# SaeedRahmani/AV-Simulation-at-Intersections

Hardware: AMD Instinct MI355X
Metric: MPC steps/sec (batch x horizon) at N=20 nu=2 (higher is better)
Workload: dtype f64

## Files before the change

av-simulation-at-intersections_amd/csrc/jsim_mpc.hip:

```cpp
#include <hip/hip_runtime.h>
#include <dlfcn.h>

#include <algorithm>
#include <cmath>
#include <cstdarg>
#include <cstdint>
#include <cstdio>
#include <cstdlib>
#include <cstring>
#include <new>
#include <type_traits>
#include <vector>

#include "jsim_mpc.h"

#define JSIM_VIOL_TOL 1e-10
#define JSIM_KEY_MASK 0xFFFFF
__device__ __forceinline__ double jsim_key_trunc(double k)
{
    return __hiloint2double(__double2hiint(k), __double2loint(k) & ~JSIM_KEY_MASK);
}
__device__ __forceinline__ double jsim_ratio_trunc(double t)
{
    return __hiloint2double(__double2hiint(t), __double2loint(t) & ~127);
// ... 9 lines not shown
#define JSIM_DEP_TOL 1e-18
#define JSIM_ACT_TOL 1e-9
#define JSIM_FEAS_TOL 1e-8

typedef double v4d __attribute__((ext_vector_type(4)));

struct KP {
    int T, n, ld, B;
    int pass;
    double dt, dl, L, w_perp, w_para;
    double R0, R1, Rd0, Rd1, Qv, Qyaw, Qf0, Qf1, Qf2, Qf3, Re0, Re1;
    double dmax, amax, amin, smax, vmax_plant, vmin, vref_min;
    double jerkw;
    const double2 *pxy;
    const double *pyaw;
    const double *pcv;
    const int *cv_cut;
    const double *pe;
    const long long *poff;
    const double *x0;
    const int *path_id;
    const int *path_len;
    const double *speed;
    long long *target_ind;
    double *oa, *od, *ox, *oy, *ov, *oyaw, *xref;
    unsigned *amask;
    int *status;
    int *n_iter;
    double *dbg_xbar;
    long long *dbg_idx;
// ... 1144 lines not shown
    {
        if (grew) *grew = n > cap;
        if (n <= cap) return hipSuccess;
        release();
        const hipError_t e = hipMalloc(&p, sizeof(T) * n);
        if (e == hipSuccess) cap = n; else p = nullptr;
        return e;
    }
};

struct jsim_ctx {
    jsim_cfg cfg{};
    int device = 0;
    DevArray<double2> d_pxy;
    DevArray<double> d_pyaw;
    DevArray<long long> d_poff;
    int n_paths = 0;
    long long n_points = 0;
    double *h_cx = nullptr, *h_cy = nullptr, *h_cyaw = nullptr;
    int have_geom = 0;
    double cc0 = 0, cc1 = 0, col_radius = 0;
    DevArray<double> d_get_all;
    DevArray<double2> d_pred_all;
    DevArray<double4> d_bc_all;
    DevArray<double4> d_pred_bc;
    double occ0 = 0, occ1 = 0, ocol_radius = 0, oL = 0;
    int have_ogeom = 0;
    DevArray<double4> d_shapes;
    DevArray<double2> d_othr;
    std::vector<double> h_shapes;
// ... 144 lines not shown
    jsim_ctx *c = new (std::nothrow) jsim_ctx();
    if (!c) return fail(nullptr, -12, "jsim_mpc_create: out of memory");
    c->cfg = *cfg;
    c->device = device_id;
    c->lds_bytes = lds_bytes;
    const char *force = getenv("JSIM_FORCE_LDS_KERNEL");
    c->use_reg_kernel = cfg->nx == 4 && has_reg_kernel(cfg->T) && !(force && force[0] == '1');
    const char *mg = getenv("JSIM_DEBUG_MAX_GI");
    c->dbg_max_gi = mg ? atoi(mg) : -1;
    *out = c;
    return 0;
}

static void free_paths(jsim_ctx *c)
{
    c->d_pxy.release(); c->d_pyaw.release(); c->d_poff.release(); c->d_pcc.release(); c->d_pcv.release();
    delete[] c->h_cx; delete[] c->h_cy; delete[] c->h_cyaw;
    c->h_cx = c->h_cy = c->h_cyaw = nullptr;
    c->n_paths = 0; c->n_points = 0;
}

extern "C" void jsim_mpc_destroy(jsim_ctx *ctx)
{
    if (!ctx) return;
    if (ctx->comm) (void)jsim_comm_destroy(ctx);
    DeviceGuard dev_guard(ctx->device);
    free_paths(ctx);
    delete ctx;
}

static int upload_circle_centres(jsim_ctx *ctx)
{
    const long long N = ctx->n_points;
    if (N <= 0 || !ctx->h_cx) return 0;
    std::vector<double2> h((size_t)2 * N);
    for (long long i = 0; i < N; ++i) {
        const double c = std::cos(ctx->h_cyaw[i]), s = std::sin(ctx->h_cyaw[i]);
        h[2 * i].x = c * ctx->cc0 - s * 0.0 + ctx->h_cx[i];     h[2 * i].y = s * ctx->cc0 + c * 0.0 + ctx->h_cy[i];
        h[2 * i + 1].x = c * ctx->cc1 - s * 0.0 + ctx->h_cx[i]; h[2 * i + 1].y = s * ctx->cc1 + c * 0.0 + ctx->h_cy[i];
    }
    ctx->d_pcc.release();
    HIP_TRY(ctx, ctx->d_pcc.reserve(2 * N));
    HIP_TRY(ctx, hipMemcpy(ctx->d_pcc, h.data(), sizeof(double2) * 2 * N, hipMemcpyHostToDevice));
    return 0;
}

extern "C" int jsim_mpc_set_paths(jsim_ctx *ctx, const double *cx, const double *cy, const double *cyaw,
                                  const int64_t *path_off, int32_t n_paths)
{
    if (!ctx) return fail(nullptr, -22, "jsim_mpc_set_paths: null ctx");
    DeviceGuard dev_guard(ctx->device);
    JSIM_GUARD_OK(ctx);
    if (!cx || !cy || !cyaw || !path_off || n_paths < 1) return fail(ctx, -22, "jsim_mpc_set_paths: bad argument");
    if (path_off[0] != 0) return fail(ctx, -22, "jsim_mpc_set_paths: path_off[0] must be 0");
    for (int i = 0; i < n_paths; ++i)
        if (path_off[i + 1] <= path_off[i]) return fail(ctx, -22, "jsim_mpc_set_paths: path %d is empty", i);
    const long long N = path_off[n_paths];
    free_paths(ctx);
    double2 *h = new (std::nothrow) double2[N];
    if (!h) return fail(ctx, -12, "jsim_mpc_set_paths: out of host memory");
    for (long long i = 0; i < N; ++i) { h[i].x = cx[i]; h[i].y = cy[i]; }
    hipError_t e = ctx->d_pxy.reserve(N);
    if (e == hipSuccess) e = ctx->d_pyaw.reserve(N);
    if (e == hipSuccess) e = ctx->d_poff.reserve(n_paths + 1);
    if (e == hipSuccess) e = hipMemcpy(ctx->d_pxy, h, sizeof(double2) * N, hipMemcpyHostToDevice);
    if (e == hipSuccess) e = hipMemcpy(ctx->d_pyaw, cyaw, sizeof(double) * N, hipMemcpyHostToDevice);
    if (e == hipSuccess) e = hipMemcpy(ctx->d_poff, path_off, sizeof(long long) * (n_paths + 1), hipMemcpyHostToDevice);
    delete[] h;
    if (e != hipSuccess) { free_paths(ctx); return fail(ctx, -5, "jsim_mpc_set_paths: %s", hipGetErrorString(e)); }
    ctx->n_paths = n_paths;
    ctx->n_points = N;
    ctx->h_cx = new (std::nothrow) double[N]; ctx->h_cy = new (std::nothrow) double[N]; ctx->h_cyaw = new (std::nothrow) double[N];
    if (!ctx->h_cx || !ctx->h_cy || !ctx->h_cyaw) return fail(ctx, -12, "jsim_mpc_set_paths: out of host memory");
    memcpy(ctx->h_cx, cx, sizeof(double) * N); memcpy(ctx->h_cy, cy, sizeof(double) * N); memcpy(ctx->h_cyaw, cyaw, sizeof(double) * N);
    if (ctx->have_geom) return upload_circle_centres(ctx);
    return 0;
}

struct StepBufs {
    double *x0; const int32_t *path_id, *path_len; const double *speed; int64_t *target_ind;
    double *oa, *od, *ox, *oy, *ov, *oyaw, *xref; uint32_t *active_mask; int32_t *status, *n_iter;
};
struct AdvanceBufs {
// ... 41 lines not shown
}

static KP fill_kp(const jsim_ctx *ctx, int32_t B, const StepBufs &S)
{
    const jsim_cfg &c = ctx->cfg;
    KP P;
    memset(&P, 0, sizeof(P));
    P.T = c.T; P.n = jsim_nvar(c.T, c.nx == 5); P.ld = jsim_ld(P.n); P.B = B;
    P.jerkw = c.jerk_weight;
    P.dt = c.dt; P.dl = c.dl; P.L = c.L; P.w_perp = c.w_perp; P.w_para = c.w_para;
    P.R0 = c.R[0]; P.R1 = c.R[1]; P.Rd0 = c.Rd[0]; P.Rd1 = c.Rd[1]; P.Qv = c.Q_v_yaw[0]; P.Qyaw = c.Q_v_yaw[1];
    P.Qf0 = c.Qf[0] * c.T; P.Qf1 = c.Qf[1] * c.T; P.Qf2 = c.Qf[2] * c.T; P.Qf3 = c.Qf[3] * c.T;
    P.Re0 = c.R_end[0]; P.Re1 = c.R_end[1];
    P.dmax = c.max_dsteer * c.dt; P.amax = c.max_accel; P.amin = c.max_decel; P.smax = c.max_steer;
    P.vmax_plant = c.max_speed; P.vmin = c.min_speed; P.vref_min = c.min_ref_speed;
    P.pxy = ctx->d_pxy; P.pyaw = ctx->d_pyaw; P.poff = ctx->d_poff;
    P.pcv = ctx->d_pcv; P.cv_cut = ctx->cv_cut; P.pe = ctx->d_pe;
    P.x0 = S.x0; P.path_id = S.path_id; P.path_len = S.path_len; P.speed = S.speed;
    P.target_ind = (long long *)S.target_ind; P.oa = S.oa; P.od = S.od; P.ox = S.ox; P.oy = S.oy; P.ov = S.ov; P.oyaw = S.oyaw;
    P.xref = S.xref; P.amask = S.active_mask; P.status = S.status; P.n_iter = S.n_iter;
    P.dbg_clk = ctx->dbg_clk; P.dbg_max_gi = ctx->dbg_max_gi;
    return P;
}

static double jsim_sqrt_threshold(double thr)
{
    double x = thr * thr;
    while (std::sqrt(x) > thr) x = std::nextafter(x, 0.0);
    while (std::sqrt(std::nextafter(x, INFINITY)) <= thr) x = std::nextafter(x, INFINITY);
    return x;
}
// ... 1136 lines not shown
```

av-simulation-at-intersections_amd/csrc/mpc_step_reg.inc:

```

template <int CTRL>
__device__ __forceinline__ double dpp_f64(double v)
{
    int lo = __double2loint(v), hi = __double2hiint(v);
    lo = __builtin_amdgcn_update_dpp(0, lo, CTRL, 0xf, 0xf, true);
    hi = __builtin_amdgcn_update_dpp(0, hi, CTRL, 0xf, 0xf, true);
    return __hiloint2double(hi, lo);
}
template <int CTRL>
__device__ __forceinline__ int dpp_i32(int v) { return __builtin_amdgcn_update_dpp(0, v, CTRL, 0xf, 0xf, true); }

#define DPP_QP_1032 0xB1
#define DPP_QP_2301 0x4E
#define DPP_ROW_HALF_MIRROR 0x141
#define DPP_ROW_MIRROR 0x140
#define DPP_ROW_SHR(n) (0x110 + (n))

__device__ __forceinline__ double wsum_dpp(double v)
{
    v += dpp_f64<DPP_QP_1032>(v);
    v += dpp_f64<DPP_QP_2301>(v);
    v += dpp_f64<DPP_ROW_HALF_MIRROR>(v);
    v += dpp_f64<DPP_ROW_MIRROR>(v);
    return (rdlane(v, 0) + rdlane(v, 16)) + (rdlane(v, 32) + rdlane(v, 48));
// ... 295 lines not shown
    if ((int)blockIdx.x >= Pin.B) return;
    const int ego = K.order ? K.order[blockIdx.x] : (int)blockIdx.x;
    if (Pin.pe) jsim_apply_ego_cfg(P, Pin.pe, ego, Pin.T, Pin.dt);
    constexpr int N = 2 * T, NR = 3 * T + 1, LD = N + 1, TP = T + 2, MW = (8 * T + 31) / 32;
    constexpr int NTILE = (N + 15) / 16;
    constexpr bool VS = NR >= 64;
    constexpr int NW = VS ? N : NR;
    static_assert(NW < 64, "register path needs 2T+1 lanes (3T+2 with resident speed rows)");
    constexpr int NP = N + 2;
    constexpr int LDC = N + 2, CCH = 16;
    constexpr bool LCA = VS || (WPE == 2 && T > 13);
    constexpr int HLN = LCA ? N * LDC : N * LD + N * LDC;
    constexpr int PREN = PRE ? (int)((sizeof(PreScratch) + 7) / 8) : 0;
    __shared__ __attribute__((aligned(16))) double HL[HLN > PREN ? HLN : PREN];
    double *const Hm = HL;
    double *const Lc = HL + (LCA ? 0 : N * LD);
    static_assert((N * LD) % 2 == 0, "Lc stays 16-byte aligned");
    __shared__ __attribute__((aligned(16))) double gsv[2 * N];
    __shared__ __attribute__((aligned(16))) double drow12[2 * NP];
    double *const drow = drow12, *const drow2 = drow12 + NP;
    __shared__ __attribute__((aligned(16))) double dzv[NP];
    __shared__ __attribute__((aligned(16))) double vzv[NP];
    __shared__ __attribute__((aligned(16))) double rdv[NP];
    __shared__ __attribute__((aligned(16))) double UV[VS ? 2 : NR + 5];
    constexpr int TQN = (TQ_COUNT * TP + 1) & ~1 ;
    constexpr int SPH = (T + 1) & ~1, SPN = VS ? T * SPH : 0;
    static_assert(!VS || (SPN >= NR + 5 || TQN + 3 * NP >= NR + 5), "uvec fits the shared area");
    __shared__ __attribute__((aligned(16))) double SCR[(TQN + 3 * NP > SPN) ? TQN + 3 * NP : SPN];
    double *const tq = SCR, *const invc = SCR + TQN, *const gvc = SCR + TQN + NP, *const wvc = SCR + TQN + 2 * NP;
    double *const spdump = SCR;
// ... 78 lines not shown
                    if (lane0 == 0) { hb_rd[(hwave - 1) * 3 + r] = v; hb_ri[(hwave - 1) * 3 + r] = id; }
                    if (i0 == id) { b0 = b1; i0 = i1; b1 = b2; i1 = i2; b2 = INFINITY; i2 = 0x7fffffff; }
                }
            } else if (cmd == HB_HBUILD) {
                if (hwave == 1 && NTILE > 1) jsim_h_tile_row<T, 1>(tq, Hm, lane0, dt);
                else if (hwave == 2 && NTILE > 2) jsim_h_tile_row<T, 2>(tq, Hm, lane0, dt);
                else if (hwave == 3 && NTILE > 3) jsim_h_tile_row<T, 3>(tq, Hm, lane0, dt);
                if (hwave == 3) { const double gi = jsim_g_own<T>(tq, lane0, dt); if (lane0 < N) gvc[lane0] = gi; }
            } else if (cmd == HB_JBUILD && hwave == 1) {
                double Jr[N];
#define JSIM_J_WAIT(n_) jsim_spin_published(&invc[(n_) - 1])
#include "mpc_step_reg_j.inc"
#undef JSIM_J_WAIT
#pragma unroll
                for (int j = 0; j < N; j += 2) *(double2 *)&Jx[lane0 * (N + 2) + j] = double2{Jr[j], Jr[j + 1]};
            }
            __syncthreads();
        }
    }
    for (int tk = 0; tk < K.n_ticks; ++tk) {
    if (WPE == 2) {
        sx = uni(sx); sy = uni(sy); sv = uni(sv); syaw = uni(syaw); di_prev = uni(di_prev); ai_last = uni(ai_last);
        goal_xy.x = uni(goal_xy.x); goal_xy.y = uni(goal_xy.y); s0 = uni64(s0); age = uni(age);
    }
#define LANE_FENCE() do { lane = lane0; asm volatile("" : "+v"(lane)); __builtin_assume(lane >= 0 && lane < 64); } while (0)
    LANE_FENCE();
    if (PRE) {
        PreScratch &W = *reinterpret_cast<PreScratch *>(HL);
        PreP pre = Q.pre;
        pre.n_obs = pre_obs.n;
        const PreOut o = jsim_pre_tick_ego(pre, Q.pred_cc_all + ((size_t)tk * Q.pre.n_obs + pre_obs.first) * Q.pre.n_steps * 2,
                                           Q.pred_bc_all + (size_t)tk * Q.pre.n_obs + pre_obs.first, pre_othr, W, lane, ego,
                                           off, Mfull, sx, sy, sv, pre_idx, pre_prev);
        pre_st = o.status;
        if (o.status == JSIM_OK) {
            pre_idx = o.idx; pre_col = o.col;
            if (Q.speed_cutoff) pre_cut = o.path_len; else M = o.path_len;
        }
        pre_prev = Q.speed_cutoff ? Mfull : (int)M;
        LDS_SYNC();
        LANE_FENCE();
    }
    double a0n = 0.0, d0n = 0.0;
    int status = JSIM_OK;
    int hp = 0;
    bool s2_done = false;
    do {
    STAMP(0);
    double bx = sx, by = sy, bv = sv, bth = syaw, sn, cs;
    long long tind = s0;
    {
        long long len = M - s0;
        if (len < 0) len = 0;
        if (M < 1) {
            status = 3;
        } else if (len >= 3) {
            double b0 = INFINITY, b1 = INFINITY, b2 = INFINITY;
            int i0 = 0x7fffffff, i1 = 0x7fffffff, i2 = 0x7fffffff;
            const double2 *pp = P.pxy + off + s0;
            const int ilen = (int)len;
#define INSERT_PT(p_, k_)                                                                      \
// ... 47 lines not shown
            tind = s0 + 1;
        }
    }
    if (status != JSIM_OK) {
        if (lane == 0) {
            P.status[ego] = status;
            if (P.n_iter) P.n_iter[ego] = it_base;
        }
        break;
    }

    STAMP(1);
    LANE_FENCE();
    const int tl_idx = lane < T ? lane : T;
    double xr, yr, yawr, vr = 0.0;
    bool rend;
    long long ik;
    {
        const double vref = (P.vref_min > sv) ? P.vref_min : sv;
        const double cstep = fabs(vref) * dt;
        double trav = cstep;
        if (P.pass == 0) {
#pragma unroll
            for (int j = 1; j <= T; ++j)
                if (j <= tl_idx) trav = trav + cstep;
        } else {
            const double *ovp = P.ov + (size_t)ego * (T + 1);
            trav = fabs(ovp[0]) * dt;
#pragma unroll
            for (int j = 1; j <= T; ++j)
                if (j <= tl_idx) trav = trav + fabs(ovp[j]) * dt;
        }
        ik = (long long)rint(trav / P.dl) + tind;
        if (ik > M - 1) ik = M - 1;
        const double2 pr = P.pxy[off + ik];
        xr = pr.x; yr = pr.y; yawr = P.pyaw[off + ik];
        rend = (ik == M - 1);
        if (P.pcv) {
            const int cut = (PRE && Q.speed_cutoff) ? pre_cut : (P.cv_cut ? P.cv_cut[ego] : -1);
            vr = (cut < 0 || ik < cut) ? P.pcv[off + ik] : 0.0;
        }
    }
    if (speed - sv < -JSIM_FEAS_TOL || sv - P.vmin < -JSIM_FEAS_TOL) status = JSIM_INFEASIBLE;

    STAMP(2);
    LANE_FENCE();
    if (!(HELP && s2_done)) {
#include "mpc_step_reg_s2.inc"
    }
    if (P.dbg_xbar && lane <= T) {
        double *xb = P.dbg_xbar + (size_t)ego * 4 * (T + 1);
        xb[0 * (T + 1) + lane] = bx; xb[1 * (T + 1) + lane] = by;
        xb[2 * (T + 1) + lane] = bv; xb[3 * (T + 1) + lane] = bth;
    }
    if (P.dbg_idx && lane <= T) P.dbg_idx[(size_t)ego * (T + 1) + lane] = ik;
    if (P.xref && lane <= T) {
        double *xf = P.xref + (size_t)ego * 4 * (T + 1);
        xf[0 * (T + 1) + lane] = xr; xf[1 * (T + 1) + lane] = yr;
        xf[2 * (T + 1) + lane] = vr; xf[3 * (T + 1) + lane] = yawr;
    }
    if (status == JSIM_INFEASIBLE) {
        if (tl) { P.oa[(size_t)ego * T + lane] = 0.0; P.od[(size_t)ego * T + lane] = 0.0; }
        wa_t = 0.0; wd_t = 0.0; s0 = tind;
        if (P.amask && lane < MW) P.amask[(size_t)ego * MW + lane] = 0u;
        if (lane == 0) {
            P.status[ego] = status;
            P.target_ind[ego] = tind;
            if (P.n_iter) P.n_iter[ego] = it_base;
        }
        break;
    }

    STAMP(3);
    LANE_FENCE();
    double al = 0, be = 0, alp = 0, bep = 0, ccx = 0, ccy = 0, kt = 0;
    if (tl) {
        al = dt * cs;
        be = (-dt * bv) * sn;
        alp = dt * sn;
        bep = (dt * bv) * cs;
        ccx = ((dt * bv) * sn) * bth;
        ccy = ((-dt * bv) * cs) * bth;
        kt = (dt * bv) / P.L;
    }
    {
        const double PA = wexscan_dpp(al, lane), PB = wexscan_dpp(be, lane);
        const double PAP = wexscan_dpp(alp, lane), PBP = wexscan_dpp(bep, lane);
        const double FX = sx + wexscan_dpp(fma(al, sv, fma(be, syaw, ccx)), lane);
        const double FY = sy + wexscan_dpp(fma(alp, sv, fma(bep, syaw, ccy)), lane);
        double Qxx = 0, Qxy = 0, Qyy = 0, qv = 0, qyaw = 0;
        if (lane >= 1 && lane <= T) {
            if (!rend) {
                const double a1 = yawr + 0.5 * M_PI;
                double c1, s1, c2, s2;
                sincos(a1, &s1, &c1); sincos(yawr, &s2, &c2);
                Qxx = (c1 * c1) * P.w_perp + (c2 * c2) * P.w_para;
                Qxy = (c1 * s1) * P.w_perp + (c2 * s2) * P.w_para;
                Qyy = (s1 * s1) * P.w_perp + (s2 * s2) * P.w_para;
                qv = P.Qv; qyaw = P.Qyaw;
            } else {
                Qxx = P.Qf0; Qyy = P.Qf1; qv = P.Qf2; qyaw = P.Qf3;
            }
        }
        const double ex = FX - xr, ey = FY - yr, ev = sv - vr, eyaw = syaw - yawr;
        if (lane <= T + 1) {
            const int t = lane;
            const bool in = lane <= T;
            tq[TQ_PA * TP + t] = PA; tq[TQ_PB * TP + t] = PB; tq[TQ_PAP * TP + t] = PAP; tq[TQ_PBP * TP + t] = PBP;
            tq[TQ_KT * TP + t] = kt;
            tq[TQ_QXX * TP + t] = in ? Qxx : 0; tq[TQ_QXY * TP + t] = in ? Qxy : 0; tq[TQ_QYY * TP + t] = in ? Qyy : 0;
// ... 245 lines not shown
        }
        LDS_SYNC();
        {
            const int rb = evl ? (lane >> 1) * NP : 0;
            double n0 = 0.0, n1 = 0.0;
#pragma unroll
            for (int j = 0; j < N; j += 2) {
                const double2 p2 = *(const double2 *)&HL[rb + j];
                n0 = fma(p2.x, p2.x, n0); n1 = fma(p2.y, p2.y, n1);
            }
            spw = (dt * dt) * (n0 + n1);
        }
        LDS_SYNC();
    }
    double *const Rm = Hm;
    for (int e = lane; e < N * LD; e += 64) Rm[e] = 0.0;
    if (lane < N) { gsv[2 * lane] = 1.0; gsv[2 * lane + 1] = 0.0; }
    if (lane < 2) { drow[N + lane] = 0.0; drow2[N + lane] = 0.0; dzv[N + lane] = 0.0; vzv[N + lane] = 0.0; }
    LDS_SYNC();

    STAMP(9);
    LANE_FENCE();
    int cid0 = -1, cid1 = -1, cid2 = -1, cid3 = -1;
    double ub0 = 0.0, lb1 = 0.0;
    const double dmx = P.dmax;
    double thr0 = 0, thr1 = 0, thr23 = 0;
    double ub2 = dmx, lb3 = -dmx, thr3 = 0;
    if (lane < N) {
        const int t = lane >> 1;
        if ((lane & 1) == 0) {
            cid0 = 4 * T + t; cid1 = 5 * T + t;
            ub0 = P.amax; lb1 = P.amin;
            thr0 = JSIM_VIOL_TOL * (1.0 + fabs(P.amax)); thr1 = JSIM_VIOL_TOL * (1.0 + fabs(P.amin));
// ... 6 lines not shown
            cid0 = 6 * T + 2 * t; cid1 = cid0 + 1;
            ub0 = P.smax; lb1 = -P.smax;
            thr0 = thr1 = JSIM_VIOL_TOL * (1.0 + P.smax);
            if (t + 1 < T) { cid2 = 2 * t; cid3 = 2 * t + 1; }
            thr23 = thr3 = JSIM_VIOL_TOL * (1.0 + P.dmax);
        }
    } else if (!VS && lane < NR && lane > N) {
        const int t = lane - N;
        cid0 = 2 * T - 2 + t; cid1 = 3 * T - 1 + t;
        ub0 = speed; lb1 = P.vmin;
        thr0 = JSIM_VIOL_TOL * (1.0 + fabs(speed - sv)); thr1 = JSIM_VIOL_TOL * (1.0 + fabs(sv - P.vmin));
    }
    double iw01, iw23, w01, w23;
    {
        double rn0 = 0.0, rn1 = 0.0, dn0 = 0.0, dn1 = 0.0;
#pragma unroll
        for (int j = 0; j < N; j += 2) {
            rn0 = fma(Jr[j], Jr[j], rn0); rn1 = fma(Jr[j + 1], Jr[j + 1], rn1);
            const double e0 = __shfl_down(Jr[j], 2) - Jr[j], e1 = __shfl_down(Jr[j + 1], 2) - Jr[j + 1];
            dn0 = fma(e0, e0, dn0); dn1 = fma(e1, e1, dn1);
        }
        const double rn = rn0 + rn1;
        const double dn = (VS && lane < N && !(lane & 1)) ? spw : dn0 + dn1;
        w01 = rn > 0.0 ? rn : 1.0;
        w23 = dn > 0.0 ? dn : 1.0;
        iw01 = fast_rcp(w01);
        iw23 = fast_rcp(w23);
    }

    int q = 0, iters = 0;
    constexpr int max_iters = 50 * N + 100;
#ifdef JSIM_STAMPS
    long long gclk[8] = {0, 0, 0, 0, 0, 0, 0, 0}, gt0 = 0, gt1 = 0;
#define GSTAMP0() do { gt0 = (long long)__builtin_readcyclecounter(); } while (0)
#define GSTAMP(i) do { gt1 = (long long)__builtin_readcyclecounter(); gclk[i] += gt1 - gt0; gt0 = gt1; } while (0)
// ... 346 lines not shown
    }
#undef JSIM_SEARCH
#undef JSIM_SEARCH_A
#undef JSIM_SEARCH_B1
#undef JSIM_SEARCH_B2
#undef JSIM_SEARCH_C

    STAMP(10);
#ifdef JSIM_STAMPS
    if (P.dbg_clk && lane == 0)
        for (int i_ = 0; i_ < 8; ++i_) P.dbg_clk[(size_t)P.B * 16 + (size_t)ego * 8 + i_] = gclk[i_];
#endif
    LANE_FENCE();
    if (status != JSIM_OK) {
        if (tl) { P.oa[(size_t)ego * T + lane] = 0.0; P.od[(size_t)ego * T + lane] = 0.0; }
        wa_t = 0.0; wd_t = 0.0; s0 = tind;
        if (P.amask && lane < MW) P.amask[(size_t)ego * MW + lane] = 0u;
        if (lane == 0) {
            P.status[ego] = status;
            P.target_ind[ego] = tind;
            if (P.n_iter) P.n_iter[ego] = it_base + iters;
            if (K.work) K.work[ego] += (unsigned)iters;
            if (K.iters) K.iters[ego] += (unsigned long long)iters;
        }
        break;
    }
    if (lane < MW) maskw[lane] = 0u;
    if (lane < (VS ? N : NR)) uvec[lane] = val;
    if (VS) {
        const bool evl = lane < N && !(lane & 1);
        const double vsp = fma(dt, wincscan_dpp(evl ? val : 0.0, lane), sv);
// ... 13 lines not shown
        if (P.amask && lane < MW) P.amask[(size_t)ego * MW + lane] = maskw[lane];
    }
    {
        double a = 0.0, dl_ = 0.0;
        if (tl) { a = uvec[2 * lane]; dl_ = uvec[2 * lane + 1]; }
        const double vt = lane <= T ? uvec[N + lane] : sv;
        if (PARK && lane <= T) {
            al = tq[TQ_QXX * TP + lane]; be = tq[TQ_QXY * TP + lane]; alp = tq[TQ_QYY * TP + lane];
            bep = tq[TQ_QV * TP + lane]; ccx = tq[TQ_QYAW * TP + lane]; ccy = tq[TQ_QEX * TP + lane]; kt = tq[TQ_KT * TP + lane];
        }
        const double yt = syaw + wexscan_dpp(kt * dl_, lane);
        const double xt = sx + wexscan_dpp(fma(al, vt, fma(be, yt, ccx)), lane);
        const double yy = sy + wexscan_dpp(fma(alp, vt, fma(bep, yt, ccy)), lane);
        if (tl) { P.oa[(size_t)ego * T + lane] = a; P.od[(size_t)ego * T + lane] = dl_; }
        wa_t = a; wd_t = dl_; s0 = tind;
        a0n = uvec[0]; d0n = uvec[1];
        if (lane <= T) {
            const size_t o = (size_t)ego * (T + 1) + lane;
            if (P.ox) P.ox[o] = xt;
            if (P.oy) P.oy[o] = yy;
            if (P.ov) P.ov[o] = vt;
            if (P.oyaw) P.oyaw[o] = yt;
        }
    }
    if (lane == 0) {
        P.status[ego] = JSIM_OK;
        P.target_ind[ego] = tind;
        if (P.n_iter) P.n_iter[ego] = it_base + iters;
        if (K.work) K.work[ego] += (unsigned)iters;
        if (K.iters) K.iters[ego] += (unsigned long long)iters;
// ... 11 lines not shown
        double di = di_prev, ai;
        if (status == JSIM_OK) { di = d0n; ai = a0n; }
        else ai = P.amin;
        di_prev = di;
        ai_last = ai;
        if (K.hist && lane == 0) {
            const int k = hist_base + tk;
            if (k < K.hist_cap) { K.hist[((size_t)k * P.B + ego) * 2] = di; K.hist[((size_t)k * P.B + ego) * 2 + 1] = ai; }
        }
        if (K.rec && lane == 0 && *K.tick + tk < K.rec_cap)
            jsim_rec_store_dev(K.rec, *K.tick + tk, P.B, ego,
                               status == JSIM_OK ? jsim_xref_deviation(P.pxy[off + s0], P.pyaw[off + s0], sx, sy) : __builtin_nan(""));
        double dc = (P.smax < di) ? P.smax : di;
        dc = (-P.smax > dc) ? -P.smax : dc;
        double cy_, sy_;
        sincos(syaw, &sy_, &cy_);
        const double xd = sv * cy_, yd = sv * sy_, thd = (sv / P.L) * tan(dc);
        sx += xd * dt; sy += yd * dt; syaw += thd * dt;
        sv += ai * dt;
        sv = (P.vmax_plant < sv) ? P.vmax_plant : sv;
        sv = (P.vmin > sv) ? P.vmin : sv;
        bool isgoal = hypot(sx - goal_xy.x, sy - goal_xy.y) <= K.goal_dis;
        long long df = s0 - M;
        if ((df < 0 ? -df : df) >= 5) isgoal = false;
        const bool done = (isgoal && fabs(sv) <= K.stop_speed) || (age + 1 >= K.max_age);
        if (K.rec && lane == 0) {
            const int k = *K.tick + tk;
            if (k < K.rec_cap)
                jsim_rec_store(K.rec, K.rec_flags, k, P.B, ego, sx, sy, syaw, sv, di, ai,
                               (status == JSIM_OK ? 0 : JSIM_REC_FAILED) | (isgoal && fabs(sv) <= K.stop_speed ? JSIM_REC_GOAL : 0) |
                                   (age + 1 >= K.max_age ? JSIM_REC_AGE : 0));
        }
        if (done) {
            sx = K.x0_spawn[4 * ego]; sy = K.x0_spawn[4 * ego + 1]; sv = K.x0_spawn[4 * ego + 2]; syaw = K.x0_spawn[4 * ego + 3];
            s0 = K.target_spawn[ego];
            wa_t = 0.0; wd_t = 0.0; di_prev = 0.0; ai_last = 0.0; age = 0;
            if (PRE) { pre_idx = 0; pre_prev = -1; }
            if (tl) { P.oa[(size_t)ego * T + lane] = 0.0; P.od[(size_t)ego * T + lane] = 0.0; }
            if (lane == 0) {
                P.target_ind[ego] = s0;
                if (K.n_respawn) atomicAdd(K.n_respawn, 1ull);
            }
        } else {
            age += 1;
        }
    }
    LDS_SYNC();
    }
    if (HELP) {
        if (lane0 == 0) hb_cmd = HB_EXIT;
        __syncthreads();
// ... 16 lines not shown
```

av-simulation-at-intersections_amd/csrc/mpc_step_reg4.inc:

```

__host__ __device__ constexpr int jsim_tile_wave4(int ntile, int a)
{
    return ntile == 5 ? (a == 0 || a == 4 ? 0 : a) : (a & 3);
}

__device__ __forceinline__ double pair_swap(double v)
{
    double r = dpp_f64<DPP_QP_1032>(v);
    asm volatile("" : "+v"(r));
    return r;
}

#ifndef JSIM_REG4_MINW
#define JSIM_REG4_MINW 2
#endif

template <int T, bool PRE>
__global__ __launch_bounds__(256, JSIM_REG4_MINW) void mpc_step_reg4_kernel(const KP P, const TickP K, const PreK Q)
{
    constexpr int N = 2 * T, NH = T, NR = 3 * T + 1, LD = N + 2, TP = T + 2, MW = (8 * T + 31) / 32, NP = N + 2;
    constexpr int NTILE = (N + 15) / 16;
    constexpr int G1 = 31, G2 = 61;
    constexpr int S2 = 64 + (N - G2);
    constexpr int SW = S2 + T + 1;
// ... 56 lines not shown
    if (PRE) {
        pre_obs = traffic_slice(Q.traffic, ego, Q.pre.n_obs);
        pre_obs.first = uni(pre_obs.first); pre_obs.n = uni(pre_obs.n);
        if (Q.pre.othr) pre_othr = Q.pre.othr + pre_obs.first;
        pre_idx = Q.traj_idx[ego];
        pre_prev = Q.prev_len[ego];
        Mfull = (int)(gp(Pv.poff)[pid + 1] - off);
        if (Q.speed_cutoff) pre_cut = Q.cut_io[ego];
    }
    const double speed = uni(gp(Pv.speed)[ego]);
    const double dt = uni((double)Pv.dt);
#define tl (lane < T)
    long long s0 = uni64(gp(Pv.target_ind)[ego]);
    double sx = gp(Pv.x0)[4 * ego + 0], sy = gp(Pv.x0)[4 * ego + 1], sv = gp(Pv.x0)[4 * ego + 2], syaw = gp(Pv.x0)[4 * ego + 3];
#define WS_SET(a_, d_) do { if (wave == 0 && tl) { wsv[0][lane] = (a_); wsv[1][lane] = (d_); } } while (0)
    WS_SET(gp(Pv.oa)[(size_t)ego * T + lane], gp(Pv.od)[(size_t)ego * T + lane]);
    __syncthreads();
    double di_prev = advance ? gp(Kv.di_ai)[2 * ego] : 0.0;
    double ai_last = advance ? gp(Kv.di_ai)[2 * ego + 1] : 0.0;
    int age = advance ? uni(gp(Kv.age)[ego]) : 0;
    const int hist_base = (advance && (Kv.hist || Kv.rec)) ? uni(*gp(Kv.tick)) : 0;
    double2 goal_xy = double2{0.0, 0.0};
    if (advance) { const jsim_d2v gq = ((JSIM_GAS const jsim_d2v *)Pv.pxy)[gp(Pv.poff)[pid + 1] - 1]; goal_xy = double2{uni(gq.x), uni(gq.y)}; }

    for (int tk = 0; tk < n_ticks; ++tk) {
#define LANE_FENCE4() do { unsigned ones_ = ~0u; asm volatile("" : "+s"(ones_)); gl = (wave << 6) | (int)__builtin_amdgcn_mbcnt_hi(ones_, __builtin_amdgcn_mbcnt_lo(ones_, 0u)); asm volatile("" : "+v"(gl)); __builtin_assume(gl >= 0 && gl < 256); lane = gl & 63; } while (0)
    LANE_FENCE4();
    sx = uni(sx); sy = uni(sy); sv = uni(sv); syaw = uni(syaw); di_prev = uni(di_prev); ai_last = uni(ai_last);
    s0 = uni64(s0); M = uni64(M); age = uni(age);
    if (PRE) {
        PreScratch &W = *reinterpret_cast<PreScratch *>(Hm);
// ... 1 lines not shown
        pre.n_obs = pre_obs.n;
        const PreOut o = jsim_pre_tick_ego<true>(pre, Q.pred_cc_all + ((size_t)tk * Q.pre.n_obs + pre_obs.first) * Q.pre.n_steps * 2,
                                           Q.pred_bc_all + (size_t)tk * Q.pre.n_obs + pre_obs.first, pre_othr, W, lane, ego,
                                           off, Mfull, sx, sy, sv, pre_idx, pre_prev);
        pre_st = o.status;
        if (o.status == JSIM_OK) {
            pre_idx = o.idx; pre_col = o.col;
            if (Q.speed_cutoff) pre_cut = o.path_len; else M = o.path_len;
        }
        pre_prev = Q.speed_cutoff ? Mfull : (int)M;
        BLOCK_SYNC();
        LANE_FENCE4();
    }
    double a0n = 0.0, d0n = 0.0;
    int status = JSIM_OK;
    do {
    STAMP2(0);
    long long tind = s0;
    {
        long long len = M - s0;
        if (len < 0) len = 0;
        if (M < 1) {
            status = 3;
        } else if (len >= 3) {
            double b0 = INFINITY, b1 = INFINITY, b2 = INFINITY;
            int i0 = 0x7fffffff, i1 = 0x7fffffff, i2 = 0x7fffffff;
            JSIM_GAS const jsim_d2v *pp = (JSIM_GAS const jsim_d2v *)Pv.pxy + off + s0;
            const int ilen = (int)len;
#define INSERT_PT(p_, k_)                                                                      \
    {                                                                                          \
// ... 33 lines not shown
        }
    }
    tind = uni64(tind);
    if (status != JSIM_OK) {
        if (gl == 0) {
            gp(Pv.status)[ego] = status;
            if (Pv.n_iter) gp(Pv.n_iter)[ego] = it_base;
        }
        break;
    }

    LANE_FENCE4();
    STAMP2(1);
    const int tl_idx = lane < T ? lane : T;
    double xr, yr, yawr, vr = 0.0;
    bool rend;
    long long ik;
    {
        const double vref = (Pv.vref_min > sv) ? Pv.vref_min : sv;
        const double cstep = fabs(vref) * dt;
        double trav = cstep;
        if (pass == 0) {
#pragma unroll
            for (int j = 1; j <= T; ++j)
                if (j <= tl_idx) trav = trav + cstep;
        } else {
            JSIM_GAS const double *ovp = gp((const double *)Pv.ov) + (size_t)ego * (T + 1);
            trav = fabs(ovp[0]) * dt;
#pragma unroll
            for (int j = 1; j <= T; ++j)
                if (j <= tl_idx) trav = trav + fabs(ovp[j]) * dt;
        }
        ik = (long long)rint(trav / Pv.dl) + tind;
        if (ik > M - 1) ik = M - 1;
        const jsim_d2v pr = ((JSIM_GAS const jsim_d2v *)Pv.pxy)[off + ik];
        xr = pr.x; yr = pr.y; yawr = gp(Pv.pyaw)[off + ik];
        rend = (ik == M - 1);
        if (Pv.pcv) {
            const int cut = (PRE && Q.speed_cutoff) ? pre_cut : (Pv.cv_cut ? gp(Pv.cv_cut)[ego] : -1);
            vr = (cut < 0 || ik < cut) ? gp(Pv.pcv)[off + ik] : 0.0;
        }
    }
    if (speed - sv < -JSIM_FEAS_TOL || sv - Pv.vmin < -JSIM_FEAS_TOL) status = JSIM_INFEASIBLE;
    status = uni(status);

    LANE_FENCE4();
    STAMP2(2);
    double bx = sx, by = sy, bv = sv, bth = syaw, sn, cs;
    {
        const double smax_ = Pv.smax, vmaxp_ = Pv.vmax_plant, vmin_ = Pv.vmin;
        const double wa_t = tl ? wsv[0][lane] : 0.0, wd_t = tl ? wsv[1][lane] : 0.0;
        double dc = (smax_ < wd_t) ? smax_ : wd_t;
        dc = (-smax_ > dc) ? -smax_ : dc;
        const double tan_t = tan(dc);
        double vcur = sv;
#pragma unroll
        for (int j = 0; j < T; ++j) {
            double vn = vcur + rdlane(wa_t, j) * dt;
            vn = (vmaxp_ < vn) ? vmaxp_ : vn;
            vn = (vmin_ > vn) ? vmin_ : vn;
            vcur = vn;
            if (lane == j + 1) bv = vn;
        }
        const double w = ((bv / Pv.L) * tan_t) * dt;
        double thcur = syaw;
#pragma unroll
        for (int j = 0; j < T; ++j) {
            thcur = thcur + rdlane(w, j);
            if (lane == j + 1) bth = thcur;
        }
        sincos(bth, &sn, &cs);
        const double ix = (bv * cs) * dt, iy = (bv * sn) * dt;
        double xcur = sx, ycur = sy;
#pragma unroll
        for (int j = 0; j < T; ++j) {
            xcur = xcur + rdlane(ix, j);
            ycur = ycur + rdlane(iy, j);
            if (lane == j + 1) { bx = xcur; by = ycur; }
        }
    }
    if (wave == 0) {
        if (Pv.dbg_xbar && lane <= T) {
            double *xb = Pv.dbg_xbar + (size_t)ego * 4 * (T + 1);
            xb[0 * (T + 1) + lane] = bx; xb[1 * (T + 1) + lane] = by;
            xb[2 * (T + 1) + lane] = bv; xb[3 * (T + 1) + lane] = bth;
        }
        if (Pv.dbg_idx && lane <= T) Pv.dbg_idx[(size_t)ego * (T + 1) + lane] = ik;
        if (Pv.xref && lane <= T) {
            JSIM_GAS double *xf = gp((double *)Pv.xref) + (size_t)ego * 4 * (T + 1);
            xf[0 * (T + 1) + lane] = xr; xf[1 * (T + 1) + lane] = yr;
            xf[2 * (T + 1) + lane] = vr; xf[3 * (T + 1) + lane] = yawr;
        }
    }
    if (status == JSIM_INFEASIBLE) {
        LANE_FENCE4();
// ... 21 lines not shown
        ccy = ((-dt * bv) * cs) * bth;
        kt = (dt * bv) / Pv.L;
    }
    if (wave == 0) {
        park[0][lane] = al; park[1][lane] = be; park[2][lane] = alp; park[3][lane] = bep;
        park[4][lane] = ccx; park[5][lane] = ccy; park[6][lane] = kt;
    }
    {
        const double PA = wexscan_dpp(al, lane), PB = wexscan_dpp(be, lane);
        const double PAP = wexscan_dpp(alp, lane), PBP = wexscan_dpp(bep, lane);
        const double FX = sx + wexscan_dpp(fma(al, sv, fma(be, syaw, ccx)), lane);
        const double FY = sy + wexscan_dpp(fma(alp, sv, fma(bep, syaw, ccy)), lane);
        double Qxx = 0, Qxy = 0, Qyy = 0, qv = 0, qyaw = 0;
        if (lane >= 1 && lane <= T) {
            if (!rend) {
                const double a1 = yawr + 0.5 * M_PI;
                double c1, s1, c2, s2;
                sincos(a1, &s1, &c1); sincos(yawr, &s2, &c2);
                Qxx = (c1 * c1) * Pv.w_perp + (c2 * c2) * Pv.w_para;
                Qxy = (c1 * s1) * Pv.w_perp + (c2 * s2) * Pv.w_para;
                Qyy = (s1 * s1) * Pv.w_perp + (s2 * s2) * Pv.w_para;
                qv = Pv.Qv; qyaw = Pv.Qyaw;
            } else {
                Qxx = Pv.Qf0; Qyy = Pv.Qf1; qv = Pv.Qf2; qyaw = Pv.Qf3;
            }
        }
        const double ex = FX - xr, ey = FY - yr, ev = sv - vr, eyaw = syaw - yawr;
        if (wave == 0 && lane <= T + 1) {
            const int t = lane;
            const bool in = lane <= T;
            tq[TQ_PA * TP + t] = PA; tq[TQ_PB * TP + t] = PB; tq[TQ_PAP * TP + t] = PAP; tq[TQ_PBP * TP + t] = PBP;
            tq[TQ_KT * TP + t] = kt;
            tq[TQ_QXX * TP + t] = in ? Qxx : 0; tq[TQ_QXY * TP + t] = in ? Qxy : 0; tq[TQ_QYY * TP + t] = in ? Qyy : 0;
// ... 836 lines not shown
            }
        }
        BLOCK_SYNC();
        if (Pv.amask && gl < MW) gp(Pv.amask)[(size_t)ego * MW + gl] = maskw[gl];
    }
    {
        const double al = park[0][lane], be = park[1][lane], alp = park[2][lane], bep = park[3][lane];
        const double ccx = park[4][lane], ccy = park[5][lane], kt = park[6][lane];
        double a = 0.0, dl_ = 0.0;
        if (tl) { a = uvec[2 * lane]; dl_ = uvec[2 * lane + 1]; }
        const double vt = lane <= T ? uvec[N + lane] : sv;
        const double yt = syaw + wexscan_dpp(kt * dl_, lane);
        const double xt = sx + wexscan_dpp(fma(al, vt, fma(be, yt, ccx)), lane);
        const double yy = sy + wexscan_dpp(fma(alp, vt, fma(bep, yt, ccy)), lane);
        if (wave == 0 && tl) { gp(Pv.oa)[(size_t)ego * T + lane] = a; gp(Pv.od)[(size_t)ego * T + lane] = dl_; }
        WS_SET(a, dl_); s0 = tind;
        a0n = uvec[0]; d0n = uvec[1];
        if (wave == 0 && lane <= T) {
            const size_t o = (size_t)ego * (T + 1) + lane;
            if (Pv.ox) gp(Pv.ox)[o] = xt;
            if (Pv.oy) gp(Pv.oy)[o] = yy;
            if (Pv.ov) gp(Pv.ov)[o] = vt;
            if (Pv.oyaw) gp(Pv.oyaw)[o] = yt;
        }
    }
    if (gl == 0) {
        gp(Pv.status)[ego] = JSIM_OK;
        gp(Pv.target_ind)[ego] = tind;
        if (Pv.n_iter) gp(Pv.n_iter)[ego] = it_base + iters;
        if (Kv.work) gp(Kv.work)[ego] += (unsigned)iters;
            if (Kv.iters) gp(Kv.iters)[ego] += (unsigned long long)iters;
// ... 7 lines not shown
        else ai = Pv.amin;
        di_prev = di;
        ai_last = ai;
        if (Kv.hist && gl == 0) {
            const int k = hist_base + tk;
            if (k < Kv.hist_cap) { gp(Kv.hist)[((size_t)k * Pv.B + ego) * 2] = di; gp(Kv.hist)[((size_t)k * Pv.B + ego) * 2 + 1] = ai; }
        }
        if (Kv.rec && gl == 0 && hist_base + tk < Kv.rec_cap) {
            const jsim_d2v rq = ((JSIM_GAS const jsim_d2v *)Pv.pxy)[off + s0];
            jsim_rec_store_dev(gp(Kv.rec), hist_base + tk, Pv.B, ego,
                               status == JSIM_OK ? jsim_xref_deviation(double2{rq.x, rq.y}, gp(Pv.pyaw)[off + s0], sx, sy)
                                                 : __builtin_nan(""));
        }
        double dc = (Pv.smax < di) ? Pv.smax : di;
        dc = (-Pv.smax > dc) ? -Pv.smax : dc;
        const double xd = sv * cos(syaw), yd = sv * sin(syaw), thd = (sv / Pv.L) * tan(dc);
        sx += xd * dt; sy += yd * dt; syaw += thd * dt;
        sv += ai * dt;
        sv = (Pv.vmax_plant < sv) ? Pv.vmax_plant : sv;
        sv = (Pv.vmin > sv) ? Pv.vmin : sv;
        bool isgoal = hypot(sx - goal_xy.x, sy - goal_xy.y) <= Kv.goal_dis;
        long long df = s0 - M;
        if ((df < 0 ? -df : df) >= 5) isgoal = false;
        const bool goal = isgoal && fabs(sv) <= Kv.stop_speed, aged = age + 1 >= Kv.max_age;
        const bool done = uni((int)(goal || aged)) != 0;
        if (Kv.rec && gl == 0) {
            const int k = hist_base + tk;
            if (k < Kv.rec_cap)
                jsim_rec_store(gp(Kv.rec), gp(Kv.rec_flags), k, Pv.B, ego, sx, sy, syaw, sv, di, ai,
                               (status == JSIM_OK ? 0 : JSIM_REC_FAILED) | (goal ? JSIM_REC_GOAL : 0) | (aged ? JSIM_REC_AGE : 0));
        }
// ... 16 lines not shown
    if (advance && gl == 0) {
        gp(Kv.x0w)[4 * ego] = sx; gp(Kv.x0w)[4 * ego + 1] = sy; gp(Kv.x0w)[4 * ego + 2] = sv; gp(Kv.x0w)[4 * ego + 3] = syaw;
        gp(Kv.di_ai)[2 * ego] = di_prev;
        gp(Kv.di_ai)[2 * ego + 1] = ai_last;
        gp(Kv.age)[ego] = age;
    }
    if (PRE && gl == 0) {
        Q.traj_idx[ego] = pre_idx;
        Q.prev_len[ego] = pre_prev;
        if (Q.speed_cutoff) Q.cut_io[ego] = pre_cut; else Q.path_len_out[ego] = (int)M;
        Q.col_flag[ego] = pre_col;
        Q.pre_status[ego] = pre_st;
    }
#undef LANE_FENCE4
#undef WS_SET
#undef tl
#undef SLOT_OF_ROW
#undef SLOTMAP4
}
```

av-simulation-at-intersections_amd/csrc/mpc_step_reg_s2.inc:

```
    {
        double dc = (P.smax < wd_t) ? P.smax : wd_t;
        dc = (-P.smax > dc) ? -P.smax : dc;
        const double tan_t = tan(dc);
        double vcur = sv;
#pragma unroll
        for (int j = 0; j < T; ++j) {
            double vn = vcur + rdlane(wa_t, j) * dt;
            vn = (P.vmax_plant < vn) ? P.vmax_plant : vn;
            vn = (P.vmin > vn) ? P.vmin : vn;
            vcur = vn;
            if (lane == j + 1) bv = vn;
        }
        const double w = ((bv / P.L) * tan_t) * dt;
        constexpr bool S2WIN = T >= 16;
        if (!S2WIN) {
        double thcur = syaw;
#pragma unroll
        for (int j = 0; j < T; ++j) {
            thcur = thcur + rdlane(w, j);
            if (lane == j + 1) bth = thcur;
        }
        sincos(bth, &sn, &cs);
        const double ix = (bv * cs) * dt, iy = (bv * sn) * dt;
        double xcur = sx, ycur = sy;
// ... 33 lines not shown
```

Before: 4.604 million.

## Precompute path yaw trig table and reuse steering tangent and heading sincos across ticks

Result: faster. 4.763 million, median of 6 (+3.4%).

```diff
diff --git a/av-simulation-at-intersections_amd/csrc/jsim_mpc.hip b/av-simulation-at-intersections_amd/csrc/jsim_mpc.hip
--- a/av-simulation-at-intersections_amd/csrc/jsim_mpc.hip
+++ b/av-simulation-at-intersections_amd/csrc/jsim_mpc.hip
@@ -47,6 +47,7 @@
     double jerkw;
     const double2 *pxy;
     const double *pyaw;
+    const double4 *ptrig;
     const double *pcv;
     const int *cv_cut;
     const double *pe;
@@ -1221,6 +1222,7 @@
     int device = 0;
     DevArray<double2> d_pxy;
     DevArray<double> d_pyaw;
+    DevArray<double4> d_ptrig;
     DevArray<long long> d_poff;
     int n_paths = 0;
     long long n_points = 0;
@@ -1395,7 +1397,7 @@
 
 static void free_paths(jsim_ctx *c)
 {
-    c->d_pxy.release(); c->d_pyaw.release(); c->d_poff.release(); c->d_pcc.release(); c->d_pcv.release();
+    c->d_pxy.release(); c->d_pyaw.release(); c->d_ptrig.release(); c->d_poff.release(); c->d_pcc.release(); c->d_pcv.release();
     delete[] c->h_cx; delete[] c->h_cy; delete[] c->h_cyaw;
     c->h_cx = c->h_cy = c->h_cyaw = nullptr;
     c->n_paths = 0; c->n_points = 0;
@@ -1424,6 +1426,17 @@
     HIP_TRY(ctx, ctx->d_pcc.reserve(2 * N));
     HIP_TRY(ctx, hipMemcpy(ctx->d_pcc, h.data(), sizeof(double2) * 2 * N, hipMemcpyHostToDevice));
     return 0;
+}
+
+__global__ __launch_bounds__(256) void path_trig_kernel(const double *pyaw, double4 *ptrig, long long n)
+{
+    const long long i = (long long)blockIdx.x * 256 + threadIdx.x;
+    if (i >= n) return;
+    const double yawr = pyaw[i];
+    const double a1 = yawr + 0.5 * M_PI;
+    double c1, s1, c2, s2;
+    sincos(a1, &s1, &c1); sincos(yawr, &s2, &c2);
+    ptrig[i] = double4{c1, s1, c2, s2};
 }
 
 extern "C" int jsim_mpc_set_paths(jsim_ctx *ctx, const double *cx, const double *cy, const double *cyaw,
@@ -1448,6 +1461,15 @@
     if (e == hipSuccess) e = hipMemcpy(ctx->d_pyaw, cyaw, sizeof(double) * N, hipMemcpyHostToDevice);
     if (e == hipSuccess) e = hipMemcpy(ctx->d_poff, path_off, sizeof(long long) * (n_paths + 1), hipMemcpyHostToDevice);
     delete[] h;
+    const char *pt = getenv("JSIM_PATH_TRIG");
+    if (e == hipSuccess && !(pt && pt[0] == '0')) {
+        e = ctx->d_ptrig.reserve(N);
+        if (e == hipSuccess) {
+            hipLaunchKernelGGL(path_trig_kernel, dim3((unsigned)((N + 255) / 256)), dim3(256), 0, 0, ctx->d_pyaw.p, ctx->d_ptrig.p, N);
+            e = hipGetLastError();
+            if (e == hipSuccess) e = hipDeviceSynchronize();
+        }
+    }
     if (e != hipSuccess) { free_paths(ctx); return fail(ctx, -5, "jsim_mpc_set_paths: %s", hipGetErrorString(e)); }
     ctx->n_paths = n_paths;
     ctx->n_points = N;
@@ -1519,7 +1541,7 @@
     P.Re0 = c.R_end[0]; P.Re1 = c.R_end[1];
     P.dmax = c.max_dsteer * c.dt; P.amax = c.max_accel; P.amin = c.max_decel; P.smax = c.max_steer;
     P.vmax_plant = c.max_speed; P.vmin = c.min_speed; P.vref_min = c.min_ref_speed;
-    P.pxy = ctx->d_pxy; P.pyaw = ctx->d_pyaw; P.poff = ctx->d_poff;
+    P.pxy = ctx->d_pxy; P.pyaw = ctx->d_pyaw; P.ptrig = ctx->d_ptrig; P.poff = ctx->d_poff;
     P.pcv = ctx->d_pcv; P.cv_cut = ctx->cv_cut; P.pe = ctx->d_pe;
     P.x0 = S.x0; P.path_id = S.path_id; P.path_len = S.path_len; P.speed = S.speed;
     P.target_ind = (long long *)S.target_ind; P.oa = S.oa; P.od = S.od; P.ox = S.ox; P.oy = S.oy; P.ov = S.ov; P.oyaw = S.oyaw;
diff --git a/av-simulation-at-intersections_amd/csrc/mpc_step_reg.inc b/av-simulation-at-intersections_amd/csrc/mpc_step_reg.inc
--- a/av-simulation-at-intersections_amd/csrc/mpc_step_reg.inc
+++ b/av-simulation-at-intersections_amd/csrc/mpc_step_reg.inc
@@ -333,6 +333,7 @@
     constexpr int PREN = PRE ? (int)((sizeof(PreScratch) + 7) / 8) : 0;
     __shared__ __attribute__((aligned(16))) double HL[HLN > PREN ? HLN : PREN];
     double *const Hm = HL;
+    constexpr bool HCLR = HELP && !LCA;
     double *const Lc = HL + (LCA ? 0 : N * LD);
     static_assert((N * LD) % 2 == 0, "Lc stays 16-byte aligned");
     __shared__ __attribute__((aligned(16))) double gsv[2 * N];
@@ -441,9 +442,19 @@
 #undef JSIM_J_WAIT
 #pragma unroll
                 for (int j = 0; j < N; j += 2) *(double2 *)&Jx[lane0 * (N + 2) + j] = double2{Jr[j], Jr[j + 1]};
+            } else if (cmd == HB_JBUILD && HCLR) {
+                for (int e = (hwave - 2) * 64 + lane0; e < N * LD; e += 128) Hm[e] = 0.0;
+                if (hwave == 2 && lane0 < N) { gsv[2 * lane0] = 1.0; gsv[2 * lane0 + 1] = 0.0; }
+                if (hwave == 3 && lane0 < 2) { drow[N + lane0] = 0.0; drow2[N + lane0] = 0.0; dzv[N + lane0] = 0.0; vzv[N + lane0] = 0.0; }
             }
             __syncthreads();
         }
+    }
+    double wtan;
+    {
+        double dc = (P.smax < wd_t) ? P.smax : wd_t;
+        dc = (-P.smax > dc) ? -P.smax : dc;
+        wtan = tan(dc);
     }
     for (int tk = 0; tk < K.n_ticks; ++tk) {
     if (WPE == 2) {
@@ -472,6 +483,8 @@
     int status = JSIM_OK;
     int hp = 0;
     bool s2_done = false;
+    double p_sn = 0.0, p_cs = 0.0;
+    bool p_sc = false;
     do {
     STAMP(0);
     double bx = sx, by = sy, bv = sv, bth = syaw, sn, cs;
@@ -549,6 +562,7 @@
     LANE_FENCE();
     const int tl_idx = lane < T ? lane : T;
     double xr, yr, yawr, vr = 0.0;
+    double4 ytr = double4{0.0, 0.0, 0.0, 0.0};
     bool rend;
     long long ik;
     {
@@ -570,6 +584,7 @@
         if (ik > M - 1) ik = M - 1;
         const double2 pr = P.pxy[off + ik];
         xr = pr.x; yr = pr.y; yawr = P.pyaw[off + ik];
+        if (P.ptrig) ytr = P.ptrig[off + ik];
         rend = (ik == M - 1);
         if (P.pcv) {
             const int cut = (PRE && Q.speed_cutoff) ? pre_cut : (P.cv_cut ? P.cv_cut[ego] : -1);
@@ -583,6 +598,7 @@
     if (!(HELP && s2_done)) {
 #include "mpc_step_reg_s2.inc"
     }
+    p_sn = rdlane(sn, 0); p_cs = rdlane(cs, 0); p_sc = true;
     if (P.dbg_xbar && lane <= T) {
         double *xb = P.dbg_xbar + (size_t)ego * 4 * (T + 1);
         xb[0 * (T + 1) + lane] = bx; xb[1 * (T + 1) + lane] = by;
@@ -596,7 +612,7 @@
     }
     if (status == JSIM_INFEASIBLE) {
         if (tl) { P.oa[(size_t)ego * T + lane] = 0.0; P.od[(size_t)ego * T + lane] = 0.0; }
-        wa_t = 0.0; wd_t = 0.0; s0 = tind;
+        wa_t = 0.0; wd_t = 0.0; wtan = 0.0; s0 = tind;
         if (P.amask && lane < MW) P.amask[(size_t)ego * MW + lane] = 0u;
         if (lane == 0) {
             P.status[ego] = status;
@@ -626,9 +642,11 @@
         double Qxx = 0, Qxy = 0, Qyy = 0, qv = 0, qyaw = 0;
         if (lane >= 1 && lane <= T) {
             if (!rend) {
-                const double a1 = yawr + 0.5 * M_PI;
-                double c1, s1, c2, s2;
-                sincos(a1, &s1, &c1); sincos(yawr, &s2, &c2);
+                double c1 = ytr.x, s1 = ytr.y, c2 = ytr.z, s2 = ytr.w;
+                if (!P.ptrig) {
+                    const double a1 = yawr + 0.5 * M_PI;
+                    sincos(a1, &s1, &c1); sincos(yawr, &s2, &c2);
+                }
                 Qxx = (c1 * c1) * P.w_perp + (c2 * c2) * P.w_para;
                 Qxy = (c1 * s1) * P.w_perp + (c2 * s2) * P.w_para;
                 Qyy = (s1 * s1) * P.w_perp + (s2 * s2) * P.w_para;
@@ -904,9 +922,11 @@
         LDS_SYNC();
     }
     double *const Rm = Hm;
-    for (int e = lane; e < N * LD; e += 64) Rm[e] = 0.0;
-    if (lane < N) { gsv[2 * lane] = 1.0; gsv[2 * lane + 1] = 0.0; }
-    if (lane < 2) { drow[N + lane] = 0.0; drow2[N + lane] = 0.0; dzv[N + lane] = 0.0; vzv[N + lane] = 0.0; }
+    if (!HCLR) {
+        for (int e = lane; e < N * LD; e += 64) Rm[e] = 0.0;
+        if (lane < N) { gsv[2 * lane] = 1.0; gsv[2 * lane + 1] = 0.0; }
+        if (lane < 2) { drow[N + lane] = 0.0; drow2[N + lane] = 0.0; dzv[N + lane] = 0.0; vzv[N + lane] = 0.0; }
+    }
     LDS_SYNC();
 
     STAMP(9);
@@ -943,11 +963,29 @@
     double iw01, iw23, w01, w23;
     {
         double rn0 = 0.0, rn1 = 0.0, dn0 = 0.0, dn1 = 0.0;
+        if (HELP) {
+            const double *const Jn = Jx + (cid2 >= 0 ? lane + 2 : lane) * (N + 2);
+#pragma unroll
+            for (int h = 0; h < N; h += CCH) {
+                double2 nb[CCH / 2];
+#pragma unroll
+                for (int j = h; j < h + CCH && j < N; j += 2) nb[(j - h) / 2] = *(const double2 *)&Jn[j];
+                JSIM_STAGE();
+#pragma unroll
+                for (int j = h; j < h + CCH && j < N; j += 2) {
+                    rn0 = fma(Jr[j], Jr[j], rn0); rn1 = fma(Jr[j + 1], Jr[j + 1], rn1);
+                    const double e0 = nb[(j - h) / 2].x - Jr[j], e1 = nb[(j - h) / 2].y - Jr[j + 1];
+                    dn0 = fma(e0, e0, dn0); dn1 = fma(e1, e1, dn1);
+                }
+                JSIM_STAGE();
+            }
+        } else {
 #pragma unroll
         for (int j = 0; j < N; j += 2) {
             rn0 = fma(Jr[j], Jr[j], rn0); rn1 = fma(Jr[j + 1], Jr[j + 1], rn1);
             const double e0 = __shfl_down(Jr[j], 2) - Jr[j], e1 = __shfl_down(Jr[j + 1], 2) - Jr[j + 1];
             dn0 = fma(e0, e0, dn0); dn1 = fma(e1, e1, dn1);
+        }
         }
         const double rn = rn0 + rn1;
         const double dn = (VS && lane < N && !(lane & 1)) ? spw : dn0 + dn1;
@@ -1324,7 +1362,7 @@
     LANE_FENCE();
     if (status != JSIM_OK) {
         if (tl) { P.oa[(size_t)ego * T + lane] = 0.0; P.od[(size_t)ego * T + lane] = 0.0; }
-        wa_t = 0.0; wd_t = 0.0; s0 = tind;
+        wa_t = 0.0; wd_t = 0.0; wtan = 0.0; s0 = tind;
         if (P.amask && lane < MW) P.amask[(size_t)ego * MW + lane] = 0u;
         if (lane == 0) {
             P.status[ego] = status;
@@ -1368,6 +1406,11 @@
         const double yy = sy + wexscan_dpp(fma(alp, vt, fma(bep, yt, ccy)), lane);
         if (tl) { P.oa[(size_t)ego * T + lane] = a; P.od[(size_t)ego * T + lane] = dl_; }
         wa_t = a; wd_t = dl_; s0 = tind;
+        if (K.advance || tk + 1 < K.n_ticks) {
+            double dc = (P.smax < dl_) ? P.smax : dl_;
+            dc = (-P.smax > dc) ? -P.smax : dc;
+            wtan = tan(dc);
+        }
         a0n = uvec[0]; d0n = uvec[1];
         if (lane <= T) {
             const size_t o = (size_t)ego * (T + 1) + lane;
@@ -1409,8 +1452,15 @@
         double dc = (P.smax < di) ? P.smax : di;
         dc = (-P.smax > dc) ? -P.smax : dc;
         double cy_, sy_;
-        sincos(syaw, &sy_, &cy_);
-        const double xd = sv * cy_, yd = sv * sy_, thd = (sv / P.L) * tan(dc);
+        if (p_sc) {
+            sy_ = syaw == 0.0 ? syaw : p_sn; cy_ = p_cs;
+        } else {
+            sincos(syaw, &sy_, &cy_);
+        }
+        double tn_;
+        if (status == JSIM_OK) tn_ = rdlane(wtan, 0);
+        else tn_ = tan(dc);
+        const double xd = sv * cy_, yd = sv * sy_, thd = (sv / P.L) * tn_;
         sx += xd * dt; sy += yd * dt; syaw += thd * dt;
         sv += ai * dt;
         sv = (P.vmax_plant < sv) ? P.vmax_plant : sv;
@@ -1429,7 +1479,7 @@
         if (done) {
             sx = K.x0_spawn[4 * ego]; sy = K.x0_spawn[4 * ego + 1]; sv = K.x0_spawn[4 * ego + 2]; syaw = K.x0_spawn[4 * ego + 3];
             s0 = K.target_spawn[ego];
-            wa_t = 0.0; wd_t = 0.0; di_prev = 0.0; ai_last = 0.0; age = 0;
+            wa_t = 0.0; wd_t = 0.0; wtan = 0.0; di_prev = 0.0; ai_last = 0.0; age = 0;
             if (PRE) { pre_idx = 0; pre_prev = -1; }
             if (tl) { P.oa[(size_t)ego * T + lane] = 0.0; P.od[(size_t)ego * T + lane] = 0.0; }
             if (lane == 0) {
diff --git a/av-simulation-at-intersections_amd/csrc/mpc_step_reg4.inc b/av-simulation-at-intersections_amd/csrc/mpc_step_reg4.inc
--- a/av-simulation-at-intersections_amd/csrc/mpc_step_reg4.inc
+++ b/av-simulation-at-intersections_amd/csrc/mpc_step_reg4.inc
@@ -94,7 +94,12 @@
     long long s0 = uni64(gp(Pv.target_ind)[ego]);
     double sx = gp(Pv.x0)[4 * ego + 0], sy = gp(Pv.x0)[4 * ego + 1], sv = gp(Pv.x0)[4 * ego + 2], syaw = gp(Pv.x0)[4 * ego + 3];
 #define WS_SET(a_, d_) do { if (wave == 0 && tl) { wsv[0][lane] = (a_); wsv[1][lane] = (d_); } } while (0)
-    WS_SET(gp(Pv.oa)[(size_t)ego * T + lane], gp(Pv.od)[(size_t)ego * T + lane]);
+#define WS_TAN(d_, out_) do { const double sm_ = Pv.smax; double dc_ = (sm_ < (d_)) ? sm_ : (d_); dc_ = (-sm_ > dc_) ? -sm_ : dc_; out_ = tan(dc_); } while (0)
+    {
+        double wt0 = 0.0;
+        if (wave == 0 && tl) { const double od0 = gp(Pv.od)[(size_t)ego * T + lane]; WS_TAN(od0, wt0); }
+        WS_SET(gp(Pv.oa)[(size_t)ego * T + lane], wt0);
+    }
     __syncthreads();
     double di_prev = advance ? gp(Kv.di_ai)[2 * ego] : 0.0;
     double ai_last = advance ? gp(Kv.di_ai)[2 * ego + 1] : 0.0;
@@ -126,6 +131,9 @@
     }
     double a0n = 0.0, d0n = 0.0;
     int status = JSIM_OK;
+    double p_sn = 0.0, p_cs = 0.0;
+    bool p_sc = false;
+    double p_tn = 0.0;
     do {
     STAMP2(0);
     long long tind = s0;
@@ -189,6 +197,7 @@
     STAMP2(1);
     const int tl_idx = lane < T ? lane : T;
     double xr, yr, yawr, vr = 0.0;
+    v4d ytr = v4d{0.0, 0.0, 0.0, 0.0};
     bool rend;
     long long ik;
     {
@@ -210,6 +219,7 @@
         if (ik > M - 1) ik = M - 1;
         const jsim_d2v pr = ((JSIM_GAS const jsim_d2v *)Pv.pxy)[off + ik];
         xr = pr.x; yr = pr.y; yawr = gp(Pv.pyaw)[off + ik];
+        if (Pv.ptrig) ytr = ((JSIM_GAS const v4d *)Pv.ptrig)[off + ik];
         rend = (ik == M - 1);
         if (Pv.pcv) {
             const int cut = (PRE && Q.speed_cutoff) ? pre_cut : (Pv.cv_cut ? gp(Pv.cv_cut)[ego] : -1);
@@ -223,11 +233,9 @@
     STAMP2(2);
     double bx = sx, by = sy, bv = sv, bth = syaw, sn, cs;
     {
-        const double smax_ = Pv.smax, vmaxp_ = Pv.vmax_plant, vmin_ = Pv.vmin;
-        const double wa_t = tl ? wsv[0][lane] : 0.0, wd_t = tl ? wsv[1][lane] : 0.0;
-        double dc = (smax_ < wd_t) ? smax_ : wd_t;
-        dc = (-smax_ > dc) ? -smax_ : dc;
-        const double tan_t = tan(dc);
+        const double vmaxp_ = Pv.vmax_plant, vmin_ = Pv.vmin;
+        const double wa_t = tl ? wsv[0][lane] : 0.0;
+        const double tan_t = tl ? wsv[1][lane] : 0.0;
         double vcur = sv;
 #pragma unroll
         for (int j = 0; j < T; ++j) {
@@ -254,6 +262,7 @@
             if (lane == j + 1) { bx = xcur; by = ycur; }
         }
     }
+    p_sn = rdlane(sn, 0); p_cs = rdlane(cs, 0); p_sc = true;
     if (wave == 0) {
         if (Pv.dbg_xbar && lane <= T) {
             double *xb = Pv.dbg_xbar + (size_t)ego * 4 * (T + 1);
@@ -305,9 +314,11 @@
         double Qxx = 0, Qxy = 0, Qyy = 0, qv = 0, qyaw = 0;
         if (lane >= 1 && lane <= T) {
             if (!rend) {
-                const double a1 = yawr + 0.5 * M_PI;
-                double c1, s1, c2, s2;
-                sincos(a1, &s1, &c1); sincos(yawr, &s2, &c2);
+                double c1 = ytr.x, s1 = ytr.y, c2 = ytr.z, s2 = ytr.w;
+                if (!Pv.ptrig) {
+                    const double a1 = yawr + 0.5 * M_PI;
+                    sincos(a1, &s1, &c1); sincos(yawr, &s2, &c2);
+                }
                 Qxx = (c1 * c1) * Pv.w_perp + (c2 * c2) * Pv.w_para;
                 Qxy = (c1 * s1) * Pv.w_perp + (c2 * s2) * Pv.w_para;
                 Qyy = (s1 * s1) * Pv.w_perp + (s2 * s2) * Pv.w_para;
@@ -1174,7 +1185,10 @@
         const double xt = sx + wexscan_dpp(fma(al, vt, fma(be, yt, ccx)), lane);
         const double yy = sy + wexscan_dpp(fma(alp, vt, fma(bep, yt, ccy)), lane);
         if (wave == 0 && tl) { gp(Pv.oa)[(size_t)ego * T + lane] = a; gp(Pv.od)[(size_t)ego * T + lane] = dl_; }
-        WS_SET(a, dl_); s0 = tind;
+        double tn = 0.0;
+        if (advance || tk + 1 < n_ticks) WS_TAN(dl_, tn);
+        p_tn = rdlane(tn, 0);
+        WS_SET(a, tn); s0 = tind;
         a0n = uvec[0]; d0n = uvec[1];
         if (wave == 0 && lane <= T) {
             const size_t o = (size_t)ego * (T + 1) + lane;
@@ -1212,7 +1226,12 @@
         }
         double dc = (Pv.smax < di) ? Pv.smax : di;
         dc = (-Pv.smax > dc) ? -Pv.smax : dc;
-        const double xd = sv * cos(syaw), yd = sv * sin(syaw), thd = (sv / Pv.L) * tan(dc);
+        double cy_ = p_cs, sy_ = p_sn;
+        if (!p_sc) { cy_ = cos(syaw); sy_ = sin(syaw); }
+        double tn_;
+        if (status == JSIM_OK) tn_ = p_tn;
+        else tn_ = tan(dc);
+        const double xd = sv * cy_, yd = sv * sy_, thd = (sv / Pv.L) * tn_;
         sx += xd * dt; sy += yd * dt; syaw += thd * dt;
         sv += ai * dt;
         sv = (Pv.vmax_plant < sv) ? Pv.vmax_plant : sv;
@@ -1259,6 +1278,7 @@
     }
 #undef LANE_FENCE4
 #undef WS_SET
+#undef WS_TAN
 #undef tl
 #undef SLOT_OF_ROW
 #undef SLOTMAP4
diff --git a/av-simulation-at-intersections_amd/csrc/mpc_step_reg_s2.inc b/av-simulation-at-intersections_amd/csrc/mpc_step_reg_s2.inc
--- a/av-simulation-at-intersections_amd/csrc/mpc_step_reg_s2.inc
+++ b/av-simulation-at-intersections_amd/csrc/mpc_step_reg_s2.inc
@@ -1,7 +1,5 @@
     {
-        double dc = (P.smax < wd_t) ? P.smax : wd_t;
-        dc = (-P.smax > dc) ? -P.smax : dc;
-        const double tan_t = tan(dc);
+        const double tan_t = wtan;
         double vcur = sv;
 #pragma unroll
         for (int j = 0; j < T; ++j) {
```
